# tepextepex/ENRGY

Measured on NVIDIA B200. Metric: cell-timesteps/s, higher is better.
Workload: dtype f32

## Files before the change

enrgy_b200/csrc/api.cu:

```cuda
#include <cuda_runtime.h>

#include <algorithm>
#include <cmath>
#include <cstdarg>
#include <cstdio>
#include <cstring>
#include <limits>
#include <string>
#include <thread>
#include <vector>

#include "../../include/enrgy_b200.h"
#include "common.cuh"
#include "kernels.cuh"
#include "prepass.cuh"

using namespace enrgy;

namespace {

thread_local std::string g_err;

int fail(int code, const char* fmt, ...) {
  char buf[1024];
// ... 138 lines not shown
  CU_TRY(cudaMemsetAsync(c->d_counters.p, 0, 2 * sizeof(unsigned long long), c->stream));
  CU_TRY(launch_mask_check(c->dem0, c->dem_pitch, d_other, c->pitch, c->band_row0, c->band_rows, c->cols,
                           c->d_counters.p, c->stream));
  c->launches++;
  unsigned long long h[2];
  CU_TRY(cudaMemcpyAsync(h, c->d_counters.p, sizeof(h), cudaMemcpyDeviceToHost, c->stream));
  CU_TRY(cudaStreamSynchronize(c->stream));
  if (h[0] != 0) {
    return fail(ENRGY_ERR_MASK,
                "%s is NaN at %llu cells where the DEM is valid; the reference would propagate NaN "
                "into only some of its area means there -- not supported",
                what, h[0]);
  }
  if (strict_other_valid && h[1] != 0) {
    return fail(ENRGY_ERR_MASK, "%s is valid at %llu cells where the DEM is NaN -- not supported", what,
                h[1]);
  }
  return ENRGY_OK;
}

template <typename R>
int upload_tables(enrgy_ctx* c) {
  const PrepassOutput& o = c->pre;
  const int T = c->n_steps;
  std::vector<StepRec<R>> st(T);
  for (int i = 0; i < T; ++i) {
    const StepRec<double>& s = o.steps[i];
    StepRec<R>& d = st[i];
    d.t_air = (R)s.t_air; d.lapse = (R)s.lapse; d.p_hpa = (R)s.p_hpa; d.e_aws = (R)s.e_aws;
    d.c_sens = (R)s.c_sens; d.c_lat = (R)s.c_lat; d.c_lwd = (R)s.c_lwd; d.c_lwu = (R)s.c_lwu;
    d.c_sw = (R)s.c_sw; d.c_melt = (R)s.c_melt; d.alb_w = (R)s.alb_w; d.snow_alb = (R)s.snow_alb;
    d.dsum = (R)s.dsum; d.dt = (R)s.dt; d.inv_dt = (R)s.inv_dt; d.c_lw0 = (R)s.c_lw0; d.c_lw1 = (R)s.c_lw1;
    d.dir_u = (R)s.dir_u; d.dir_e = (R)s.dir_e; d.dir_n = (R)s.dir_n;
    d.tan2_min = (R)s.tan2_min;
    if ((double)d.tan2_min > s.tan2_min) d.tan2_min = std::nextafter(d.tan2_min, (R)-1);
    const int32_t pair_code = (int32_t)s.alb_pair, sub_code = (int32_t)s.sub;
    d.alb_pair = (R)0; d.sub = (R)0;
    std::memcpy(&d.alb_pair, &pair_code, sizeof(int32_t));
    std::memcpy(&d.sub, &sub_code, sizeof(int32_t));
  }
  const size_t ns = o.subs.size();
  std::vector<SubRec<R>> sb(std::max<size_t>(ns, 1));
  for (size_t i = 0; i < ns; ++i) {
    sb[i].e = (R)o.subs[i].e; sb[i].n = (R)o.subs[i].n; sb[i].u = (R)o.subs[i].u; sb[i].b = (R)o.subs[i].b;
  }
  CU_TRY(c->d_steps.alloc(std::max<size_t>(T, 1) * sizeof(StepRec<R>)));
  CU_TRY(c->d_steps64.alloc(std::max<size_t>(T, 1)));
  CU_TRY(c->d_subs.alloc(sb.size() * sizeof(SubRec<R>)));
  CU_TRY(c->d_blocks.alloc(std::max<size_t>(o.blocks.size(), 1)));
  if (T) {
    CU_TRY(cudaMemcpyAsync(c->d_steps.p, st.data(), (size_t)T * sizeof(StepRec<R>), cudaMemcpyHostToDevice, c->stream));
    CU_TRY(cudaMemcpyAsync(c->d_steps64.p, o.steps.data(), (size_t)T * sizeof(StepRec<double>), cudaMemcpyHostToDevice, c->stream));
    CU_TRY(cudaMemcpyAsync(c->d_blocks.p, o.blocks.data(), o.blocks.size() * sizeof(TimeBlock), cudaMemcpyHostToDevice, c->stream));
  }
  if (ns) {
    CU_TRY(cudaMemcpyAsync(c->d_subs.p, sb.data(), ns * sizeof(SubRec<R>), cudaMemcpyHostToDevice, c->stream));
  }
  CU_TRY(cudaStreamSynchronize(c->stream));
  return ENRGY_OK;
}

template <typename R>
int upload_stations(enrgy_ctx* c) {
  const int T = c->n_steps;
  std::vector<StationRec<R>> recs((size_t)std::max(T, 1) * kMaxStations);
  for (int i = 0; i < T; ++i) {
    const StepRec<double>& s = c->pre.steps[i];
    StationRec<R>* r = &recs[(size_t)i * kMaxStations];
    r[0].t = (R)s.t_air; r[0].p = (R)s.p_hpa; r[0].e = (R)s.e_aws; r[0].cn = (R)0;
    const double n0 = c->forcing[(size_t)i * ENRGY_F_COUNT + ENRGY_F_CLOUD];
    for (int k = 1; k < kMaxStations; ++k) {
      if (k <= c->n_extra) {
// ... 1550 lines not shown
```

enrgy_b200/csrc/common.cuh:

```cuda
#pragma once
#include <cstdint>
#include <cmath>

#if defined(__CUDACC__)
#define ENRGY_HD __host__ __device__ __forceinline__
#else
#define ENRGY_HD inline
#endif

namespace enrgy {

constexpr double kRair = 287.058;
constexpr double kKarman = 0.4;
constexpr double kGrav = 9.81;
constexpr double kCpAir = 1010.0;
constexpr double kLv = 2.514 * 1e6;
constexpr double kSigma = 5.70 * 1e-8;
constexpr double kLf = 3.34 * 1e5;
constexpr double kCice = 2097.0;
constexpr double kKappaIce = 1.16 * 1e-6;
constexpr double kKappaSnow = 0.40 * 1e-6;
constexpr double kPressureLapse = -0.1145;
constexpr double kVapourScale = 6300.0;
constexpr double kMsmInitLapse = -0.006;

constexpr int kThreads = 256;
constexpr int kWarps = kThreads / 32;
constexpr int kTileW = 128;
constexpr int kStatsK = 8;
constexpr int kStatsM = 2;
constexpr int kStatsP = kStatsK + kStatsM;
#ifndef ENRGY_STEPS_PER_BLOCK
#define ENRGY_STEPS_PER_BLOCK 64
#endif
// ... 3 lines not shown
enum StatK { K_RS = 0, K_LWD, K_SENS, K_LAT, K_MELT, K_SNOW, K_SWE, K_NSNOW };
enum StatM { M_LWU = 0, M_G };

constexpr int kMaxLayers = 7;
template <typename R>
struct MsmParams {
  int layers;
  R d[kMaxLayers], inv_d[kMaxLayers];
  R c_ice, k_ice, k_snow, rho_ice, rho_snow;
  R inv_snow_density;
  R g0_ice;
  R crd_ice, inv_crd_ice;
};

template <typename R>
struct alignas(16) StepRec {
  R t_air;
  R lapse;
  R p_hpa;
  R e_aws;
  R c_sens;
  R c_lat;
  R c_lwd;
  R c_lwu;
  R c_sw;
  R c_melt;
  R alb_w;
  R snow_alb;
  R dsum;
  R dt;
  R alb_pair;
  R sub;
  R dir_u, dir_e, dir_n;
  R tan2_min;
  R inv_dt;
  R c_lw0;
  R c_lw1;
  R pad_;
};

constexpr int kMaxFusedMembers = 4;
template <typename R>
struct alignas(8) MemberRec {
  R c_sens, c_lat;
};

constexpr int kMaxStations = 4;
template <typename R>
struct alignas(16) StationRec {
  R t;
  R p;
  R e;
  R cn;
};

template <typename R>
struct alignas(16) SubRec {
  R e, n, u;
  R b;
};
struct alignas(16) ShadeRec {
  int32_t dc_fix;
  int32_t dr_fix;
  float dz;
  int32_t kmax;
};
ENRGY_HD void line_geometry(int dc_fix, int dr_fix, bool* row_type, int* sigma, int* dfix) {
  const int adr = dr_fix < 0 ? -dr_fix : dr_fix, adc = dc_fix < 0 ? -dc_fix : dc_fix;
  *row_type = adr >= adc;
  if (*row_type) { *sigma = dr_fix > 0 ? 1 : -1; *dfix = dc_fix; }
  else { *sigma = dc_fix > 0 ? 1 : -1; *dfix = dr_fix; }
}
// ... 9 lines not shown
```

enrgy_b200/csrc/kernels.cu:

```cuda
#include "kernels.cuh"

#include <cstdio>
#include <cstring>
#include <type_traits>

#include "../../include/enrgy_b200.h"

namespace enrgy {

__device__ __forceinline__ uint32_t smem_u32(const void* p) {
  return static_cast<uint32_t>(__cvta_generic_to_shared(p));
}
__device__ __forceinline__ void mbar_init(uint64_t* bar, unsigned count) {
  asm volatile("mbarrier.init.shared::cta.b64 [%0], %1;" ::"r"(smem_u32(bar)), "r"(count));
}
__device__ __forceinline__ void mbar_expect_tx(uint64_t* bar, unsigned bytes) {
  asm volatile("mbarrier.arrive.expect_tx.shared::cta.b64 _, [%0], %1;" ::"r"(smem_u32(bar)),
               "r"(bytes)
               : "memory");
}
__device__ __forceinline__ void mbar_wait(uint64_t* bar, unsigned parity) {
  asm volatile(
      "{\n\t"
      ".reg .pred p;\n\t"
// ... 102 lines not shown
  V2<float> d;
  asm("add.rn.f32x2 %0, %1, %2;" : "=l"(d.v) : "l"(a.v), "l"(b.v));
  return d;
}
__device__ __forceinline__ V2<float> sub2(V2<float> a, V2<float> b) {
  V2<float> d;
  asm("sub.rn.f32x2 %0, %1, %2;" : "=l"(d.v) : "l"(a.v), "l"(b.v));
  return d;
}
__device__ __forceinline__ V2<float> mul2(V2<float> a, V2<float> b) {
  V2<float> d;
  asm("mul.rn.f32x2 %0, %1, %2;" : "=l"(d.v) : "l"(a.v), "l"(b.v));
  return d;
}
__device__ __forceinline__ V2<double> fma2(V2<double> a, V2<double> b, V2<double> c) {
  return V2<double>{a.a * b.a + c.a, a.b * b.b + c.b};
}
__device__ __forceinline__ V2<double> add2(V2<double> a, V2<double> b) { return V2<double>{a.a + b.a, a.b + b.b}; }
__device__ __forceinline__ V2<double> sub2(V2<double> a, V2<double> b) { return V2<double>{a.a - b.a, a.b - b.b}; }
__device__ __forceinline__ V2<double> mul2(V2<double> a, V2<double> b) { return V2<double>{a.a * b.a, a.b * b.b}; }
__device__ __forceinline__ V2<float> lapse_product(V2<float> d, float g) {
  return V2<float>::make(__fmul_rn(d.lo(), g), __fmul_rn(d.hi(), g));
}
__device__ __forceinline__ V2<double> lapse_product(V2<double> d, double g) { return V2<double>{d.a * g, d.b * g}; }
__device__ __forceinline__ void keep_in_register(V2<float>& x) { asm volatile("" : "+l"(x.v)); }
__device__ __forceinline__ void keep_in_register(V2<double>&) {}

__device__ __forceinline__ float mul_rn(float a, float b) { return __fmul_rn(a, b); }
__device__ __forceinline__ float add_rn(float a, float b) { return __fadd_rn(a, b); }
__device__ __forceinline__ float div_rn(float a, float b) { return __fdiv_rn(a, b); }
__device__ __forceinline__ double mul_rn(double a, double b) { return __dmul_rn(a, b); }
__device__ __forceinline__ double add_rn(double a, double b) { return __dadd_rn(a, b); }
__device__ __forceinline__ double div_rn(double a, double b) { return __ddiv_rn(a, b); }
__device__ __forceinline__ float sq_sum(float x, float y) { return __fadd_rn(__fmul_rn(x, x), __fmul_rn(y, y)); }
__device__ __forceinline__ double sq_sum(double x, double y) { return __dadd_rn(__dmul_rn(x, x), __dmul_rn(y, y)); }

__device__ __forceinline__ float fmax_(float a, float b) { return fmaxf(a, b); }
__device__ __forceinline__ float fmin_(float a, float b) { return fminf(a, b); }
__device__ __forceinline__ double fmax_(double a, double b) { return fmax(a, b); }
__device__ __forceinline__ double fmin_(double a, double b) { return fmin(a, b); }

template <typename R>
__device__ __forceinline__ R warp_reduce8(const R (&v)[8], int lane) {
  const unsigned full = 0xffffffffu;
  R a[4], b[2], c;
  bool hi = (lane & 16) != 0;
#pragma unroll
  for (int i = 0; i < 4; ++i) {
    const R send = hi ? v[i] : v[i + 4];
    const R keep = hi ? v[i + 4] : v[i];
    a[i] = keep + __shfl_xor_sync(full, send, 16);
  }
  hi = (lane & 8) != 0;
#pragma unroll
  for (int i = 0; i < 2; ++i) {
    const R send = hi ? a[i] : a[i + 2];
    const R keep = hi ? a[i + 2] : a[i];
    b[i] = keep + __shfl_xor_sync(full, send, 8);
  }
  hi = (lane & 4) != 0;
  {
    const R send = hi ? b[0] : b[1];
    const R keep = hi ? b[1] : b[0];
    c = keep + __shfl_xor_sync(full, send, 4);
  }
  c += __shfl_xor_sync(full, c, 2);
  c += __shfl_xor_sync(full, c, 1);
  return c;
// ... 229 lines not shown
template <typename R>
cudaError_t launch_nan_offglacier(const float* dem, int dem_pitch, int pitch, int band_row0,
                                  int band_rows, int cols, R* swe, R* tsn, R* tic, cudaStream_t stream) {
  nan_offglacier_kernel<R><<<1184, 256, 0, stream>>>(dem, dem_pitch, pitch, band_row0, band_rows, cols, swe,
                                                     tsn, tic);
  return cudaGetLastError();
}
template cudaError_t launch_nan_offglacier<float>(const float*, int, int, int, int, int, float*, float*, float*, cudaStream_t);
template cudaError_t launch_nan_offglacier<double>(const float*, int, int, int, int, int, double*, double*, double*, cudaStream_t);

#ifndef ENRGY_WARPS32
#define ENRGY_WARPS32 4
#endif
#ifndef ENRGY_WARPS64
#define ENRGY_WARPS64 4
#endif
template <typename R, int INSOL>
constexpr int kWarpsFor = sizeof(R) == 4 ? ENRGY_WARPS32 : ENRGY_WARPS64;
__host__ __device__ constexpr int warps_x(int w) { return w >= 4 ? 4 : w; }

#ifndef ENRGY_MASK_RING
#define ENRGY_MASK_RING 0
#endif
constexpr int kRingSlots = 16, kRingAhead = 8;
__device__ __forceinline__ void cp_async16(void* smem_dst, const void* gsrc) {
  asm volatile("cp.async.cg.shared.global [%0], [%1], 16;" ::"r"(smem_u32(smem_dst)), "l"(gsrc) : "memory");
}
__device__ __forceinline__ void cp_async_commit() { asm volatile("cp.async.commit_group;" ::: "memory"); }
template <int N>
__device__ __forceinline__ void cp_async_wait() { asm volatile("cp.async.wait_group %0;" ::"n"(N) : "memory"); }

template <typename R>
struct SmemPlan {
  int steps, subs, members, stations, slots, slots_m, ring, full, total;
};
#ifndef ENRGY_ONE_BARRIER
#define ENRGY_ONE_BARRIER 1
#endif
template <typename R, bool MSM, int NM, int INSOL>
constexpr bool kOneBarrier = ENRGY_ONE_BARRIER && sizeof(R) == 4 && !MSM && NM == 1 && INSOL == kInsolMasked;

template <typename R>
__host__ __device__ inline SmemPlan<R> smem_plan(int warps, int cap_steps, int cap_subs, bool with_subs, bool msm,
                                                 int nm = 1, int ns = 1, bool with_masks = false) {
  SmemPlan<R> p;
  int o = 0;
  p.steps = o;   o += 2 * cap_steps * (int)sizeof(StepRec<R>);
  p.subs = o;    o += with_subs ? 2 * cap_subs * (int)sizeof(SubRec<R>) : 0;
  p.members = o; o += nm > 1 ? 2 * cap_steps * nm * (int)sizeof(MemberRec<R>) : 0;
  p.stations = o; o += ns > 1 ? 2 * cap_steps * ns * (int)sizeof(StationRec<R>) : 0;
  const bool two_sets = ENRGY_ONE_BARRIER && sizeof(R) == 4 && !msm && nm == 1 && with_masks;
  p.slots = o;   o += (two_sets ? 2 : 1) * warps * cap_steps * nm * kStatsK * (int)sizeof(R);
  p.slots_m = o; o += msm ? warps * cap_steps * kStatsM * (int)sizeof(R) : 0;
  o = (o + 15) / 16 * 16;
  p.ring = o;    o += (ENRGY_MASK_RING && with_masks) ? warps * kRingSlots * 32 : 0;
  p.full = o;    o += 16;
  p.total = (o + 127) / 128 * 128;
  return p;
}

#ifndef ENRGY_K32
#define ENRGY_K32 8
#endif
#ifndef ENRGY_K64
#define ENRGY_K64 4
#endif
#ifndef ENRGY_MINB32
#define ENRGY_MINB32 4
#endif
#ifndef ENRGY_MINB64
#define ENRGY_MINB64 3
#endif

#ifndef ENRGY_SUB_UNROLL
#define ENRGY_SUB_UNROLL 4
#endif
constexpr int kSubUnroll = ENRGY_SUB_UNROLL;
#ifndef ENRGY_MASK_AHEAD
#define ENRGY_MASK_AHEAD 4
#endif
constexpr int kMaskAhead = ENRGY_MASK_AHEAD;
#ifndef ENRGY_MINB_MEMBERS
#define ENRGY_MINB_MEMBERS 3
#endif
template <typename R, int K, int INSOL, bool MSM, bool DUMP, int NM = 1, int KT = K, bool STATS = true, int NS = 1>
__global__ void __launch_bounds__(32 * kWarpsFor<R, INSOL>, NM > 2 ? ENRGY_MINB_MEMBERS : sizeof(R) == 4 ? ENRGY_MINB32 : ENRGY_MINB64)
energy_balance_kernel(const KernelArgs<R> a) {
  static_assert(NM == 1 || (!MSM && !DUMP), "fused members: no sub-surface model, no dump");
  static_assert(KT % K == 0, "a patch is walked in whole parts");
  static_assert(STATS || NM > 1, "only fused members run without statistics");
  static_assert(NS == 1 || (NM == 1 && !MSM), "station blend: no fused members, no sub-surface model");
  constexpr int W = kWarpsFor<R, INSOL>;
  constexpr int WX = warps_x(W), WY = W / WX;
  constexpr int NT = 32 * W;
  extern __shared__ __align__(128) unsigned char smem_raw[];
  const int cap_steps = a.cap_steps, cap_subs = a.cap_subs;
  const SmemPlan<R> plan = smem_plan<R>(W, cap_steps, cap_subs, INSOL != kInsolStreamed, MSM, NM, NS, INSOL == kInsolMasked);
  StationRec<R>* const sm_stations = reinterpret_cast<StationRec<R>*>(smem_raw + plan.stations);
  StepRec<R>* const sm_steps = reinterpret_cast<StepRec<R>*>(smem_raw + plan.steps);
  SubRec<R>* const sm_subs = reinterpret_cast<SubRec<R>*>(smem_raw + plan.subs);
  MemberRec<R>* const sm_members = reinterpret_cast<MemberRec<R>*>(smem_raw + plan.members);
  R* const sm_slots0 = reinterpret_cast<R*>(smem_raw + plan.slots);
  constexpr bool ONE_BAR = kOneBarrier<R, MSM, NM, INSOL>;
  unsigned slot_set = 0;
  R* const sm_slots_m = reinterpret_cast<R*>(smem_raw + plan.slots_m);
  uint64_t* const sm_full = reinterpret_cast<uint64_t*>(smem_raw + plan.full);

  constexpr int TILE_H = WY * KT, TILE_W = 32 * WX;
  const int tid = threadIdx.x, lane = tid & 31, warp = tid >> 5;
  const R qnan = (R)__int_as_float(0x7fc00000);

  if (tid == 0) {
    mbar_init(&sm_full[0], 1);
    mbar_init(&sm_full[1], 1);
    fence_mbar_init();
  }
  __syncthreads();
  unsigned phase[2] = {0u, 0u};

  auto issue_block = [&](int b, int buf) {
    const TimeBlock tb = a.blocks[b];
    const unsigned n_steps = (unsigned)(tb.t_end - tb.t_begin);
    const unsigned n_subs = (unsigned)(tb.sub_end - tb.sub_begin);
    unsigned bytes = n_steps * (unsigned)sizeof(StepRec<R>);
    if (INSOL != kInsolStreamed) bytes += n_subs * (unsigned)sizeof(SubRec<R>);
    if (NM > 1) bytes += n_steps * NM * (unsigned)sizeof(MemberRec<R>);
    if (NS > 1) bytes += n_steps * NS * (unsigned)sizeof(StationRec<R>);
    fence_proxy_async();
    mbar_expect_tx(&sm_full[buf], bytes);
    tma_bulk_g2s(sm_steps + buf * cap_steps, a.steps + tb.t_begin, n_steps * (unsigned)sizeof(StepRec<R>),
// ... 83 lines not shown
        } else {
          x_[h] = y_[h] = (R)0; n_[h] = (R)1;
        }
#pragma unroll
        for (int m = 0; m < NM; ++m) {
          s_[m][h] = v ? a.swe[m * m_stride + o] : (R)0;
          t_[m][h] = v ? a.total_ice[m * m_stride + o] : (R)0;
        }
        if (MSM) {
#pragma unroll
          for (int l = 0; l < NB; ++l) {
            tl[i][l] = (v && l <= a.msm.layers) ? a.layer_t[(size_t)l * a.layer_stride + o] : (R)0;
          }
          t0_acc[i] = (double)tl[i][0];
        }
      }
      delta2[q] = V::make(d_[0], d_[1]);
      keep_in_register(delta2[q]);
#pragma unroll
      for (int k = 0; k < NS; ++k) {
        pw2[k][q] = V::make(p_[k][0], p_[k][1]);
        if (NS > 1) wst2[k][q] = V::make(w_[k][0], w_[k][1]);
      }
      nx2[q] = V::make(x_[0], x_[1]);
      ny2[q] = V::make(y_[0], y_[1]);
      nz2[q] = V::make(n_[0], n_[1]);
#pragma unroll
      for (int m = 0; m < NM; ++m) {
        swe2[m][q] = V::make(s_[m][0], s_[m][1]);
        tic2[m][q] = V::make(t_[m][0], t_[m][1]);
        om2[m][q] = V::splat(a.albedo_const ? (R)1 - m_alb_ice(m) : (R)0.5);
      }
    }
    constexpr bool kAnalyticBeam = INSOL == kInsolComputed && sizeof(R) == 4;
    R patch_g2 = (R)0;
    if (kAnalyticBeam) {
#pragma unroll
      for (int q = 0; q < KP; ++q) {
        patch_g2 = fmax_(patch_g2, fmax_(sq_sum(nx2[q].lo(), ny2[q].lo()), sq_sum(nx2[q].hi(), ny2[q].hi())));
      }
      if (KT > K) {
        const int prow0 = row0 - part * K;
        for (int i = 0; i < KT; ++i) {
          const int rowb = prow0 + i;
          if (rowb < a.band_rows && colx < a.cols && (i < part * K || i >= part * K + K)) {
            const size_t o = (size_t)rowb * a.pitch + colx;
            const R gx = a.nx[o], gy = a.ny[o];
            if (gx == gx) patch_g2 = fmax_(patch_g2, sq_sum(gx, gy));
          }
        }
      }
#pragma unroll
      for (int d = 16; d > 0; d >>= 1) patch_g2 = fmax_(patch_g2, __shfl_xor_sync(0xffffffffu, patch_g2, d));
      patch_g2 *= (R)1.00001;
    }
    keep_in_register(valid_bits);
    const bool patch_full = __all_sync(0xffffffffu, valid_bits == ((1u << K) - 1u));
    const unsigned lane_bit = 1u << lane;
    constexpr bool RING = ENRGY_MASK_RING && INSOL == kInsolMasked && K == 8;
    uint4* const ring = reinterpret_cast<uint4*>(smem_raw + plan.ring) + warp * kRingSlots * 2;
    int ring_next = -0x40000000;
    const unsigned* const mask_patch =
        INSOL == kInsolMasked
            ? a.masks + ((size_t)(row0 >> 3) * a.mask_words + (size_t)((colx - lane) >> 5)) * 8 + (row0 & 7) -
                  (size_t)a.mask_sub0 * a.mask_sub_stride
            : nullptr;

    int buf = 0;
    if (tid == 0) issue_block(a.block_begin, 0);

    for (int b = a.block_begin; b < a.block_end; ++b, buf ^= 1) {
      if (tid == 0 && b + 1 < a.block_end) issue_block(b + 1, buf ^ 1);
      R* const sm_slots = sm_slots0 + (ONE_BAR ? (size_t)(slot_set & 1u) * W * cap_steps * NM * kStatsK : 0);
      slot_set ^= 1u;
      mbar_wait(&sm_full[buf], phase[buf]);
      phase[buf] ^= 1u;
      const TimeBlock tb = a.blocks[b];
      const int ts = max(tb.t_begin, a.t0), te = min(tb.t_end, a.t1);

      float pot_next[K];
      if (INSOL == kInsolStreamed) {
#pragma unroll
        for (int i = 0; i < K; ++i) {
          const size_t o = (size_t)(ts - a.pot_t0) * a.pot_stride + (size_t)(row0 + i) * a.pitch + colx;
          pot_next[i] = (valid_bits >> i) & 1u ? __ldg(a.pot + o) : 0.f;
        }
      }

      auto run_steps = [&](auto full_tag) {
      constexpr bool FULL = decltype(full_tag)::value;
      const StepRec<R>* const steps_b = sm_steps + buf * cap_steps - tb.t_begin;
      int sub_next = step_code(steps_b[ts].sub), pair_next = step_code(steps_b[ts].alb_pair);
      R w_next = steps_b[ts].alb_w;
      for (int t = ts; t < te; ++t) {
        const StepRec<R> s = steps_b[t];
        const int sub_code = sub_next, pair = pair_next;
        const R alb_w = w_next;
        if (t + 1 < te) {
          sub_next = step_code(steps_b[t + 1].sub);
          pair_next = step_code(steps_b[t + 1].alb_pair);
          w_next = steps_b[t + 1].alb_w;
        }
        if (!a.albedo_const) {
          if (pair != cur_pair || alb_w != cur_w) {
            cur_pair = pair;
            cur_w = alb_w;
            const float* m0 = a.albedo + (size_t)(pair >> 8) * a.map_stride;
            const float* m1 = a.albedo + (size_t)(pair & 255) * a.map_stride;
#pragma unroll
            for (int q = 0; q < KP; ++q) {
              R om[NM][2];
#pragma unroll
              for (int h = 0; h < 2; ++h) {
                const int i = 2 * q + h;
                const size_t o = (size_t)(row0 + i) * a.pitch + colx;
                const bool v = (valid_bits >> i) & 1u;
                const R y0 = v ? (R)__ldg(m0 + o) : (R)0.5, y1 = v ? (R)__ldg(m1 + o) : (R)0.5;
#pragma unroll
                for (int m = 0; m < NM; ++m) {
                  const R x0 = v ? fmin_(fmax_(y0 + m_offset(m), (R)0.001f), (R)1) : (R)0.5;
                  const R x1 = v ? fmin_(fmax_(y1 + m_offset(m), (R)0.001f), (R)1) : (R)0.5;
                  om[m][h] = ((R)1 - x0) + alb_w * (x0 - x1);
                }
              }
#pragma unroll
              for (int m = 0; m < NM; ++m) om2[m][q] = V::make(om[m][0], om[m][1]);
            }
          }
        }
        float pot_cur[K];
        if (INSOL == kInsolStreamed) {
#pragma unroll
          for (int i = 0; i < K; ++i) pot_cur[i] = pot_next[i];
// ... 5 lines not shown
            }
          }
        }

        V pot2[KP];
        auto balance = [&]() {
        const V zero2 = V::splat((R)0);
        V acc_sens = zero2, acc_lat = zero2;
        V acc_lwd = zero2;
        V acc_rs[NM], acc_mf[NM], acc_snow[NM], acc_swe[NM], acc_lwu = zero2, acc_g = zero2;
        int n_snow[NM];
#pragma unroll
        for (int m = 0; m < NM; ++m) { acc_rs[m] = acc_mf[m] = acc_snow[m] = acc_swe[m] = zero2; n_snow[m] = 0; }
        const V keep_map = V::splat(s.snow_alb >= (R)0 ? (R)0 : (R)1);
        const R ice_floor = (R)1 - a.max_ice_albedo;
        const V t_aws = V::splat(s.t_air), lapse2 = V::splat(s.lapse), p_aws = V::splat(s.p_hpa), e_aws = V::splat(s.e_aws);
        const V c_lwd = V::splat(s.c_lwd), c_sw = V::splat(s.c_sw), c_melt = V::splat(s.c_melt);
        V c_sens[NM], c_lat[NM], snow_const[NM];
#pragma unroll
        for (int m = 0; m < NM; ++m) {
          if (NM > 1) {
            const MemberRec<R> mr = sm_members[(buf * cap_steps + (t - tb.t_begin)) * NM + m];
            c_sens[m] = V::splat(mr.c_sens);
            c_lat[m] = V::splat(mr.c_lat);
            const R sa = a.albedo_const ? a.member_albedo_snow[m] : s.snow_alb;
            snow_const[m] = V::splat(s.snow_alb >= (R)0 ? (R)1 - sa : (R)0);
          } else {
            c_sens[m] = V::splat(s.c_sens);
            c_lat[m] = V::splat(s.c_lat);
            snow_const[m] = V::splat(s.snow_alb >= (R)0 ? (R)1 - s.snow_alb : (R)0);
          }
        }
        const V k273 = V::splat((R)273.15), k_plapse = V::splat((R)kPressureLapse), k_rair = V::splat((R)kRair),
                k_fp0 = V::splat((R)1.0016), k_fp1 = V::splat((R)(3.15 * 1e-6)), k_fp2 = V::splat((R)-0.074);
#pragma unroll
        for (int q = 0; q < KP; ++q) {
          V t_st = t_aws, p_st = p_aws, e_st = zero2, cloud_fac = zero2;
          if (NS > 1) {
            const StationRec<R>* const sr = sm_stations + (buf * cap_steps + (t - tb.t_begin)) * NS;
            V cn = zero2;
#pragma unroll
            for (int k = 0; k < NS; ++k) {
              const StationRec<R> r = sr[k];
              if (k == 0) {
                t_st = sizeof(R) == 4 ? lapse_product(wst2[0][q], r.t) : mul2(wst2[0][q], V::splat(r.t));
                p_st = mul2(wst2[0][q], V::splat(r.p));
                e_st = mul2(pw2[0][q], V::splat(r.e));
              } else {
                t_st = sizeof(R) == 4 ? add2(t_st, lapse_product(wst2[k][q], r.t)) : fma2(wst2[k][q], V::splat(r.t), t_st);
                p_st = fma2(wst2[k][q], V::splat(r.p), p_st);
                e_st = fma2(pw2[k][q], V::splat(r.e), e_st);
                cn = k == 1 ? mul2(wst2[1][q], V::splat(r.cn)) : fma2(wst2[k][q], V::splat(r.cn), cn);
              }
            }
            if (a.cloud_on) {
              const V x = mul2(cn, V::splat(a.cloud_neg_k));
              cloud_fac = V::make(Num<R>::exp_(x.lo()), Num<R>::exp_(x.hi()));
            }
          }
          const V t_air = sizeof(R) == 4 ? add2(t_st, lapse_product(delta2[q], s.lapse)) : fma2(delta2[q], lapse2, t_st);
          const V tz = add2(t_air, k273);
          V d_t = sub2(tz, k273);
          if (MSM) {
            R d[2];
#pragma unroll
            for (int h = 0; h < 2; ++h) {
              const int i = 2 * q + h;
              const R tzh = h ? tz.hi() : tz.lo();
              d[h] = tzh - (tl[i][0] + (R)273.15);
              if (sizeof(R) == 4) {
                d[h] = ((tzh - (R)273.15) + (R)-6.103515625e-06) - tl[i][0];
              }
            }
            d_t = V::make(d[0], d[1]);
          }
          const V p_hpa = fma2(delta2[q], k_plapse, p_st);
          const V e = NS > 1 ? e_st : mul2(pw2[0][q], e_aws);
          V r_rt, r_p;
          {
            const V rt = mul2(tz, k_rair);
            if (sizeof(R) == 8) {
              const V den = mul2(rt, p_hpa);
              const V inv = V::make(Num<R>::rcp(den.lo()), Num<R>::rcp(den.hi()));
              r_rt = mul2(inv, p_hpa);
              r_p = mul2(inv, rt);
            } else {
              r_rt = V::make(Num<R>::rcp(rt.lo()), Num<R>::rcp(rt.hi()));
              r_p = V::make(Num<R>::rcp(p_hpa.lo()), Num<R>::rcp(p_hpa.hi()));
            }
          }
          const V x_sens = mul2(p_hpa, mul2(r_rt, d_t));
          const V f_p = fma2(r_p, k_fp2, fma2(p_hpa, k_fp1, k_fp0));
          V es_neg = V::splat((R)-611.2);
          if (MSM) {
            R x[2];
#pragma unroll
            for (int h = 0; h < 2; ++h) {
              const R t0 = tl[2 * q + h][0];
              x[h] = (R)-611.2 * Num<R>::exp_(((R)17.62 * t0) * Num<R>::rcp((R)243.12 + t0));
            }
            es_neg = V::make(x[0], x[1]);
          }
          const V x_lat = mul2(r_rt, fma2(es_neg, f_p, e));
          const V tzsq = mul2(tz, tz);
          const V tz4 = mul2(tzsq, tzsq);
          V lwu = V::splat(s.c_lwu);
          if (MSM) {
            R x[2];
#pragma unroll
            for (int h = 0; h < 2; ++h) {
              const R t0 = tl[2 * q + h][0];
              if (sizeof(R) == 4) {
                const R y = t0 * (R)(1.0 / 273.15);
                const R poly = (R)1 + y * ((R)4 + y * ((R)6 + y * ((R)4 + y)));
                x[h] = (s.c_lwu * (R)(273.15 * 273.15 * 273.15 * 273.15)) * poly;
              } else {
                const R ts_k = t0 + (R)273.15;
                const R ts2 = ts_k * ts_k;
                x[h] = s.c_lwu * (ts2 * ts2);
              }
            }
            lwu = V::make(x[0], x[1]);
          }
          V rl;
          if (sizeof(R) == 4 && !MSM) {
            const V y = mul2(d_t, V::splat((R)(1.0 / (double)273.15f)));
            const V poly = mul2(y, fma2(y, fma2(y, add2(y, V::splat((R)4)), V::splat((R)6)), V::splat((R)4)));
            rl = fma2(V::splat(s.c_lw1), poly, V::splat(s.c_lw0));
          } else {
            const V lwu_neg = V::make(-lwu.lo(), -lwu.hi());
            rl = fma2(c_lwd, tz4, lwu_neg);
          }
          const bool v_lo = (valid_bits >> (2 * q)) & 1u, v_hi = (valid_bits >> (2 * q + 1)) & 1u;
          if (STATS) {
            V m_sens = x_sens, m_lat = x_lat;
            if (!FULL) {
// ... 245 lines not shown
                  for (int p_ = 0; p_ < kRingAhead; ++p_) fetch(ms + p_);
                  ring_next = ms + kRingAhead;
                }
                fetch(ring_next);
                ++ring_next;
                cp_async_wait<kRingAhead>();
                __syncwarp();
                const uint4 m0 = ring[(ms & (kRingSlots - 1)) * 2], m1 = ring[(ms & (kRingSlots - 1)) * 2 + 1];
                mw[0] = m0.x; mw[1] = m0.y; mw[2 % K] = m0.z; mw[3 % K] = m0.w;
                mw[4 % K] = m1.x; mw[5 % K] = m1.y; mw[6 % K] = m1.z; mw[7 % K] = m1.w;
              } else if (K == 8) {
                const uint4 m0 = __ldg(reinterpret_cast<const uint4*>(mp)), m1 = __ldg(reinterpret_cast<const uint4*>(mp) + 1);
                mw[0] = m0.x; mw[1] = m0.y; mw[2 % K] = m0.z; mw[3 % K] = m0.w;
                mw[4 % K] = m1.x; mw[5 % K] = m1.y; mw[6 % K] = m1.z; mw[7 % K] = m1.w;
              } else if (K == 4) {
                const uint4 m0 = __ldg(reinterpret_cast<const uint4*>(mp));
                mw[0] = m0.x; mw[1] = m0.y; mw[2 % K] = m0.z; mw[3 % K] = m0.w;
              } else {
                const uint2 m0 = __ldg(reinterpret_cast<const uint2*>(mp));
                mw[0] = m0.x; mw[1] = m0.y;
              }
            }
#pragma unroll
            for (int q = 0; q < KP; ++q) {
              R c_lo = fmax_(c2[q].lo(), (R)0), c_hi = fmax_(c2[q].hi(), (R)0);
              if (INSOL == kInsolMasked) {
                c_lo = (mw[2 * q] & lane_bit) ? c_lo : (R)0;
                c_hi = (mw[2 * q + 1] & lane_bit) ? c_hi : (R)0;
              }
              direct2[q] = fma2(b2, V::make(c_lo, c_hi), direct2[q]);
            }
          };
          constexpr bool kOneBalance = MSM;
          if (kAnalyticBeam && patch_g2 < s.tan2_min) {
            const V du = V::splat(s.dir_u), de = V::splat(s.dir_e), dn = V::splat(s.dir_n);
#pragma unroll
            for (int q = 0; q < KP; ++q) direct2[q] = fma2(ny2[q], dn, fma2(nx2[q], de, du));
            if (!kOneBalance) finish_step();
          } else if (nj == 4) {
            sub_step(j0); sub_step(j0 + 1); sub_step(j0 + 2); sub_step(j0 + 3);
            if (!kOneBalance) finish_step();
          } else {
#pragma unroll(kSubUnroll)
            for (int j = j0; j < j0 + nj; ++j) sub_step(j);
            if (!kOneBalance) finish_step();
          }
          if (kOneBalance) finish_step();
        }
      }
      };
      if (patch_full) run_steps(std::true_type{}); else run_steps(std::false_type{});

      __syncthreads();
      if (!DUMP && STATS && my_partials != nullptr) {
        constexpr int NQ = MSM ? kStatsP : kStatsK;
        const int n = (te - ts) * NM * NQ;
        for (int idx = tid; idx < n; idx += NT) {
          const int step = idx / NQ, q = idx - step * NQ;
          const int sl = (ts - tb.t_begin) * NM + step;
          double sum = 0.0;
#pragma unroll
          for (int w = 0; w < W; ++w) {
            sum += q < kStatsK ? (double)sm_slots[(w * cap_steps * NM + sl) * kStatsK + q]
                               : (double)sm_slots_m[(w * cap_steps + sl) * kStatsM + (q - kStatsK)];
          }
          my_partials[((size_t)(ts - a.t0) * NM + step) * kRow + q] += (R)sum;
        }
// ... 27 lines not shown
        }
      }
    }
  }
}

template <typename R, bool MSM>
struct CellsPerThread {
  static constexpr int kBase = sizeof(R) == 4 ? ENRGY_K32 : ENRGY_K64;
  static constexpr int value = MSM ? ((kBase / 2 + 1) & ~1) : kBase;
};

template <typename R>
void energy_balance_tile(bool msm, int insol, int* tile_h, int* tile_w) {
  const int k = msm ? CellsPerThread<R, true>::value : CellsPerThread<R, false>::value;
  (void)insol;
  const int w = kWarpsFor<R, kInsolComputed>;
  *tile_w = 32 * warps_x(w);
  *tile_h = (w / warps_x(w)) * k;
}
template void energy_balance_tile<float>(bool, int, int*, int*);
template void energy_balance_tile<double>(bool, int, int*, int*);

template <typename R, bool MSM, int NM, int NS = 1>
struct PassShape {
  static constexpr int KT = CellsPerThread<R, MSM>::value;
  static constexpr int K = (NM > 1 || NS > 1) ? KT / 2 : KT;
};

template <typename R, int INSOL, bool MSM, bool DUMP, int NM = 1, bool STATS = true, int NS = 1>
static cudaError_t configure(int sm_count, int cap_steps, int cap_subs, LaunchInfo* info) {
  constexpr int K = PassShape<R, MSM, NM, NS>::K, KT = PassShape<R, MSM, NM, NS>::KT;
  auto kern = energy_balance_kernel<R, K, INSOL, MSM, DUMP, NM, KT, STATS, NS>;
  const int smem = smem_plan<R>(kWarpsFor<R, INSOL>, cap_steps, cap_subs, INSOL != kInsolStreamed, MSM, NM, NS, INSOL == kInsolMasked).total;
  cudaError_t e = cudaFuncSetAttribute(kern, cudaFuncAttributeMaxDynamicSharedMemorySize, smem);
  if (e != cudaSuccess) return e;
  int per_sm = 0;
  e = cudaOccupancyMaxActiveBlocksPerMultiprocessor(&per_sm, kern, 32 * kWarpsFor<R, INSOL>, smem);
  if (e != cudaSuccess) return e;
  cudaFuncAttributes fa;
  e = cudaFuncGetAttributes(&fa, kern);
  if (e != cudaSuccess) return e;
  if (per_sm < 1) per_sm = 1;
  info->regs = fa.numRegs;
  info->smem_bytes = smem;
  info->ctas_per_sm = per_sm;
  info->grid = per_sm * sm_count;
  info->cells_per_thread = K;
  return cudaSuccess;
}

template <typename R, int INSOL, bool MSM, bool DUMP, int NM = 1, bool STATS = true, int NS = 1>
static cudaError_t launch_one(const KernelArgs<R>& a, int sm_count, int forced_grid, LaunchInfo* info,
                              cudaStream_t stream) {
  constexpr int K = PassShape<R, MSM, NM, NS>::K, KT = PassShape<R, MSM, NM, NS>::KT;
  LaunchInfo li;
  cudaError_t e = configure<R, INSOL, MSM, DUMP, NM, STATS, NS>(sm_count, a.cap_steps, a.cap_subs, &li);
  if (e != cudaSuccess) return e;
  int grid = forced_grid > 0 ? forced_grid : li.grid;
  li.grid = grid;
  if (info) *info = li;
  if (a.n_tiles == 0 || a.t1 <= a.t0) return cudaSuccess;
  energy_balance_kernel<R, K, INSOL, MSM, DUMP, NM, KT, STATS, NS><<<grid, 32 * kWarpsFor<R, INSOL>, li.smem_bytes, stream>>>(a);
  return cudaGetLastError();
}

template <typename R, typename F>
// ... 326 lines not shown
```

enrgy_b200/csrc/prepass.cu:

```cuda
#include "prepass.cuh"

#include <algorithm>
#include <cmath>
#include <cstdio>
#include <limits>

namespace enrgy {

namespace {

constexpr double kDeg = 0.017453292519943295;
constexpr double kPi = 3.141592653589793;

constexpr double kA = 0.7, kB = 0.75, kC = 5.0, kD = 0.35;

double minus_psi_m(double z, double l) {
  const double zeta = z / l;
  if (zeta >= 0) {
    return kA * zeta + kB * (zeta - kC / kD) * std::exp(-kD * zeta) + kB * kC / kD;
  }
  const double x = std::pow(1 - 16 * zeta, 0.25);
  return -(2 * std::log((1 + x) / 2) + std::log((1 + x * x) / 2) - 2 * std::atan(x) + kPi / 2);
}

// ... 228 lines not shown
    } else {
      s.c_lwu = p.emissivity * kSigma * std::pow(ts_k, 4.0);
    }
    {
      const double k0 = (double)273.15f, k04 = (k0 * k0) * (k0 * k0);
      const double c_lwd_k = mirror32 ? (double)(float)s.c_lwd : s.c_lwd;
      s.c_lw1 = c_lwd_k * k04;
      s.c_lw0 = s.c_lw1 - (mirror32 ? (double)(float)s.c_lwu : s.c_lwu);
    }
    s.c_melt = dt / kLf / 1000;
    s.dt = dt;
    s.inv_dt = 1.0 / dt;

    const int i0 = (int)f[ENRGY_F_ALB_I0], i1 = (int)f[ENRGY_F_ALB_I1];
    const double span = f[ENRGY_F_ALB_SPAN];
    s.alb_pair = (double)(i0 * 256 + i1);
    s.alb_w = span > 0 ? f[ENRGY_F_ALB_DAYS] / span : 0.0;
    const double snow_days = f[ENRGY_F_SNOW_DAYS];
    s.snow_alb = snow_days > 0 ? 0.40 + 0.44 * std::exp(-0.12 * snow_days) : -1.0;
    if (p.albedo_const) {
      s.snow_alb = p.albedo_snow;
      s.alb_w = 0.0;
      s.alb_pair = 0.0;
    }

    double pot_aws_kwh = 0.0;
    out.sub_first[i] = (int)out.subs.size();
    if (computed) {
      const double dt_h = dt / 3600.0;
      const double hs = p.hour_step;
      int n_sub = (int)std::ceil(dt_h / hs - 1e-9);
      if (n_sub < 1) n_sub = 1;
      double direct = 0.0, dsum = 0.0;
      double dir_u = 0.0, dir_e = 0.0, dir_n = 0.0, tan2_min = std::numeric_limits<double>::infinity();
      for (int j = 0; j < n_sub; ++j) {
        const double w = std::min(hs, dt_h - j * hs);
        const double t_mid = f[ENRGY_F_TIME] + (j * hs + 0.5 * w) * 3600.0;
        SubHost sb;
        sun_vector(t_mid, p.lat_deg, p.lon_deg, &sb.e, &sb.n, &sb.u);
        if (!(sb.u > 0.0)) continue;
        const double tb = std::pow(p.transmittance, 1.0 / sb.u);
        sb.b = p.solar_const * tb * w / 1000.0;
        sb.d = p.solar_const * (0.271 - 0.294 * tb) * sb.u * w / 1000.0 * 0.5;
        const double m = std::max(std::fabs(sb.e), std::fabs(sb.n));
        if (m > 0.0) {
          sb.shade.dc_fix = (int32_t)std::floor(sb.e / m * 65536.0 + 0.5);
          sb.shade.dr_fix = (int32_t)std::floor(-sb.n / m * 65536.0 + 0.5);
          sb.shade.dz = (float)(p.cell_size * sb.u / m);
        } else {
          sb.shade.dc_fix = 0;
          sb.shade.dr_fix = 0;
          sb.shade.dz = std::numeric_limits<float>::infinity();
        }
        sb.shade.kmax = std::max(in.rows, in.cols);
        out.subs.push_back(sb);
        dir_u += sb.b * sb.u; dir_e += sb.b * sb.e; dir_n += sb.b * sb.n;
        {
          const double h2 = sb.e * sb.e + sb.n * sb.n;
          if (h2 > 0.0) tan2_min = std::min(tan2_min, sb.u * sb.u / h2);
        }
        const double cosi = nx * sb.e + ny * sb.n + nz * sb.u;
        double term = sb.b * std::max(cosi, 0.0);
        if (p.shadow && !host_lit(in.dem, in.rows, in.cols, p.aws_row, p.aws_col, sb.shade)) {
          term = 0.0;
        }
        direct = direct + term;
        dsum = dsum + sb.d;
      }
      s.dsum = dsum;
      s.dir_u = dir_u; s.dir_e = dir_e; s.dir_n = dir_n;
      s.tan2_min = (int)out.subs.size() == out.sub_first[i] ? -1.0 : std::min(tan2_min, 1e30);
      pot_aws_kwh = direct + dsum * (1.0 + nz);
    } else {
      s.dsum = 0.0;
      s.dir_u = s.dir_e = s.dir_n = 0.0; s.tan2_min = -1.0;
      pot_aws_kwh = in.pot_aws ? in.pot_aws[i] : 0.0;
    }
    out.sub_count[i] = (int)out.subs.size() - out.sub_first[i];
    if (out.sub_count[i] > 255) {
      err = "more than 255 insolation sub-steps in one time step";
      return ENRGY_ERR_RANGE;
    }

    double pot_w, factor;
    const double swd = f[ENRGY_F_SWD];
    if (mirror32 && !computed) {
      const float pw32 = (((float)pot_aws_kwh * 3.6f) * 1000000.0f) / (float)dt;
      pot_w = (double)pw32;
      factor = pw32 == 0.0f ? 1.0 : (double)((float)swd / pw32);
    } else {
      pot_w = pot_aws_kwh * 3.6 * 1000000 / dt;
      factor = pot_w == 0 ? 1.0 : swd / pot_w;
    }
    s.c_sw = 3.6 * 1000000 / dt * factor;

    const double t_air_c = t_air + delta_cell * f[ENRGY_F_LAPSE];
    const double tz_c = t_air_c + 273.15;
    const double tsk = ts_aws_c + 273.15;
    const double p_c = p_hpa + delta_cell * kPressureLapse;
    const double r_rt = 1.0 / (kRair * tz_c);
    const double sens = (s.c_sens * p_c) * (r_rt * (tz_c - tsk));
    const double f_p = 1.0016 + 3.15 * 1e-6 * p_c - 0.074 / p_c;
    const double es = 611.2 * std::exp((17.62 * ts_aws_c) / (243.12 + ts_aws_c)) * f_p;
    const double lat = (s.c_lat * r_rt) * (e_aws * pw_cell - es);
    pt[ENRGY_P_SENS_AWS] = sens;
    pt[ENRGY_P_LAT_AWS] = lat;
    if (msm) {
      for (int lyr = 0; lyr <= nl; ++lyr) out.point_layers[(size_t)i * (kMaxLayers + 1) + lyr] = tl[lyr];
// ... 82 lines not shown
```

Measured before the change: 579.0 billion.

## Use per-azimuth-sector slope bounds to take analytic beam path more often

Replaces the single patch-wide max-gradient test for skipping the shadow ray march with a per-warp table of directional slope maxima over 64 azimuth sectors at 6 arc widths. The prepass encodes each step's sun-azimuth arc as a sector code and stores the min sun tangent (not its square). The tighter bound lets more timesteps take the cheap analytic direct-beam path, at the cost of a per-warp table build and extra shared memory. It also refolds the latent-heat vapour pressure terms into fused multiply-adds for the non-MSM path.

After: 610.2 billion, median of 6. 5.4% higher.

```diff
diff --git a/enrgy_b200/csrc/api.cu b/enrgy_b200/csrc/api.cu
--- a/enrgy_b200/csrc/api.cu
+++ b/enrgy_b200/csrc/api.cu
@@ -194,12 +194,13 @@
     d.c_sw = (R)s.c_sw; d.c_melt = (R)s.c_melt; d.alb_w = (R)s.alb_w; d.snow_alb = (R)s.snow_alb;
     d.dsum = (R)s.dsum; d.dt = (R)s.dt; d.inv_dt = (R)s.inv_dt; d.c_lw0 = (R)s.c_lw0; d.c_lw1 = (R)s.c_lw1;
     d.dir_u = (R)s.dir_u; d.dir_e = (R)s.dir_e; d.dir_n = (R)s.dir_n;
-    d.tan2_min = (R)s.tan2_min;
-    if ((double)d.tan2_min > s.tan2_min) d.tan2_min = std::nextafter(d.tan2_min, (R)-1);
-    const int32_t pair_code = (int32_t)s.alb_pair, sub_code = (int32_t)s.sub;
-    d.alb_pair = (R)0; d.sub = (R)0;
+    d.tan_min = (R)s.tan_min;
+    if ((double)d.tan_min > s.tan_min) d.tan_min = std::nextafter(d.tan_min, (R)-1);
+    const int32_t pair_code = (int32_t)s.alb_pair, sub_code = (int32_t)s.sub, sector_code = (int32_t)s.sector;
+    d.alb_pair = (R)0; d.sub = (R)0; d.sector = (R)0;
     std::memcpy(&d.alb_pair, &pair_code, sizeof(int32_t));
     std::memcpy(&d.sub, &sub_code, sizeof(int32_t));
+    std::memcpy(&d.sector, &sector_code, sizeof(int32_t));
   }
   const size_t ns = o.subs.size();
   std::vector<SubRec<R>> sb(std::max<size_t>(ns, 1));
diff --git a/enrgy_b200/csrc/common.cuh b/enrgy_b200/csrc/common.cuh
--- a/enrgy_b200/csrc/common.cuh
+++ b/enrgy_b200/csrc/common.cuh
@@ -1,5 +1,6 @@
 #pragma once
 #include <cstdint>
+#include <algorithm>
 #include <cmath>
 
 #if defined(__CUDACC__)
@@ -69,12 +70,27 @@
   R alb_pair;
   R sub;
   R dir_u, dir_e, dir_n;
-  R tan2_min;
+  R tan_min;
   R inv_dt;
   R c_lw0;
   R c_lw1;
-  R pad_;
+  R sector;
 };
+
+constexpr int kSectors = 64;
+constexpr int kSectorLevels = 6;
+inline int sector_arc_code(const int* sec, int n) {
+  if (n <= 0) return -1;
+  int best_len = kSectors + 1, best_first = 0;
+  for (int i = 0; i < n; ++i) {
+    int len = 0;
+    for (int j = 0; j < n; ++j) len = std::max(len, ((sec[j] - sec[i]) % kSectors + kSectors) % kSectors + 1);
+    if (len < best_len) { best_len = len; best_first = sec[i]; }
+  }
+  int level = 0;
+  while ((1 << level) < best_len) ++level;
+  return level < kSectorLevels ? level * kSectors + best_first : -1;
+}
 
 constexpr int kMaxFusedMembers = 4;
 template <typename R>
diff --git a/enrgy_b200/csrc/kernels.cu b/enrgy_b200/csrc/kernels.cu
--- a/enrgy_b200/csrc/kernels.cu
+++ b/enrgy_b200/csrc/kernels.cu
@@ -158,8 +158,6 @@
 __device__ __forceinline__ double mul_rn(double a, double b) { return __dmul_rn(a, b); }
 __device__ __forceinline__ double add_rn(double a, double b) { return __dadd_rn(a, b); }
 __device__ __forceinline__ double div_rn(double a, double b) { return __ddiv_rn(a, b); }
-__device__ __forceinline__ float sq_sum(float x, float y) { return __fadd_rn(__fmul_rn(x, x), __fmul_rn(y, y)); }
-__device__ __forceinline__ double sq_sum(double x, double y) { return __dadd_rn(__dmul_rn(x, x), __dmul_rn(y, y)); }
 
 __device__ __forceinline__ float fmax_(float a, float b) { return fmaxf(a, b); }
 __device__ __forceinline__ float fmin_(float a, float b) { return fminf(a, b); }
@@ -455,17 +453,20 @@
 
 template <typename R>
 struct SmemPlan {
-  int steps, subs, members, stations, slots, slots_m, ring, full, total;
+  int steps, subs, members, stations, slots, slots_m, ring, sectors, full, total;
 };
 #ifndef ENRGY_ONE_BARRIER
 #define ENRGY_ONE_BARRIER 1
 #endif
+template <typename R, int INSOL>
+constexpr bool kAnalyticBeamFor = INSOL == kInsolComputed && sizeof(R) == 4;
 template <typename R, bool MSM, int NM, int INSOL>
 constexpr bool kOneBarrier = ENRGY_ONE_BARRIER && sizeof(R) == 4 && !MSM && NM == 1 && INSOL == kInsolMasked;
 
 template <typename R>
 __host__ __device__ inline SmemPlan<R> smem_plan(int warps, int cap_steps, int cap_subs, bool with_subs, bool msm,
-                                                 int nm = 1, int ns = 1, bool with_masks = false) {
+                                                 int nm = 1, int ns = 1, bool with_masks = false,
+                                                 bool with_sectors = false) {
   SmemPlan<R> p;
   int o = 0;
   p.steps = o;   o += 2 * cap_steps * (int)sizeof(StepRec<R>);
@@ -477,6 +478,7 @@
   p.slots_m = o; o += msm ? warps * cap_steps * kStatsM * (int)sizeof(R) : 0;
   o = (o + 15) / 16 * 16;
   p.ring = o;    o += (ENRGY_MASK_RING && with_masks) ? warps * kRingSlots * 32 : 0;
+  p.sectors = o; o += with_sectors ? warps * kSectorLevels * kSectors * (int)sizeof(float) : 0;
   p.full = o;    o += 16;
   p.total = (o + 127) / 128 * 128;
   return p;
@@ -518,7 +520,8 @@
   constexpr int NT = 32 * W;
   extern __shared__ __align__(128) unsigned char smem_raw[];
   const int cap_steps = a.cap_steps, cap_subs = a.cap_subs;
-  const SmemPlan<R> plan = smem_plan<R>(W, cap_steps, cap_subs, INSOL != kInsolStreamed, MSM, NM, NS, INSOL == kInsolMasked);
+  const SmemPlan<R> plan = smem_plan<R>(W, cap_steps, cap_subs, INSOL != kInsolStreamed, MSM, NM, NS, INSOL == kInsolMasked,
+                                        kAnalyticBeamFor<R, INSOL>);
   StationRec<R>* const sm_stations = reinterpret_cast<StationRec<R>*>(smem_raw + plan.stations);
   StepRec<R>* const sm_steps = reinterpret_cast<StepRec<R>*>(smem_raw + plan.steps);
   SubRec<R>* const sm_subs = reinterpret_cast<SubRec<R>*>(smem_raw + plan.subs);
@@ -668,27 +671,66 @@
         om2[m][q] = V::splat(a.albedo_const ? (R)1 - m_alb_ice(m) : (R)0.5);
       }
     }
-    constexpr bool kAnalyticBeam = INSOL == kInsolComputed && sizeof(R) == 4;
-    R patch_g2 = (R)0;
-    if (kAnalyticBeam) {
-#pragma unroll
-      for (int q = 0; q < KP; ++q) {
-        patch_g2 = fmax_(patch_g2, fmax_(sq_sum(nx2[q].lo(), ny2[q].lo()), sq_sum(nx2[q].hi(), ny2[q].hi())));
+    constexpr bool kAnalyticBeam = kAnalyticBeamFor<R, INSOL>;
+    float* const sec_tab = reinterpret_cast<float*>(smem_raw + plan.sectors) + warp * kSectorLevels * kSectors;
+    if constexpr (kAnalyticBeam) {
+      constexpr int KO = KT - K;
+      float ox[KO > 0 ? KO : 1], oy[KO > 0 ? KO : 1];
+#pragma unroll
+      for (int j = 0; j < KO; ++j) {
+        const int i = j < part * K ? j : j + K;
+        const int rowb = row0 - part * K + i;
+        ox[j] = oy[j] = 0.f;
+        if (rowb < a.band_rows && colx < a.cols) {
+          const size_t o = (size_t)rowb * a.pitch + colx;
+          const float gx = a.nx[o], gy = a.ny[o];
+          if (gx == gx) { ox[j] = gx; oy[j] = gy; }
+        }
       }
-      if (KT > K) {
-        const int prow0 = row0 - part * K;
-        for (int i = 0; i < KT; ++i) {
-          const int rowb = prow0 + i;
-          if (rowb < a.band_rows && colx < a.cols && (i < part * K || i >= part * K + K)) {
-            const size_t o = (size_t)rowb * a.pitch + colx;
-            const R gx = a.nx[o], gy = a.ny[o];
-            if (gx == gx) patch_g2 = fmax_(patch_g2, sq_sum(gx, gy));
-          }
-        }
+      float hb_lo = 0.f, hb_hi = 0.f;
+      for (int i = 0; i < kSectors / 2; ++i) {
+        float sn, cs;
+        sincospif((float)i * (2.0f / kSectors), &sn, &cs);
+        float dmin = 0.f, dmax = 0.f;
+#pragma unroll
+        for (int q = 0; q < KP; ++q) {
+          const float d0 = fmaf(nx2[q].lo(), cs, ny2[q].lo() * sn), d1 = fmaf(nx2[q].hi(), cs, ny2[q].hi() * sn);
+          dmin = fminf(dmin, fminf(d0, d1));
+          dmax = fmaxf(dmax, fmaxf(d0, d1));
+        }
+#pragma unroll
+        for (int j = 0; j < KO; ++j) {
+          const float d = fmaf(ox[j], cs, oy[j] * sn);
+          dmin = fminf(dmin, d);
+          dmax = fmaxf(dmax, d);
+        }
+#pragma unroll
+        for (int d = 16; d > 0; d >>= 1) {
+          dmin = fminf(dmin, __shfl_xor_sync(0xffffffffu, dmin, d));
+          dmax = fmaxf(dmax, __shfl_xor_sync(0xffffffffu, dmax, d));
+        }
+        if (lane == i) { hb_lo = -dmin; hb_hi = dmax; }
       }
-#pragma unroll
-      for (int d = 16; d > 0; d >>= 1) patch_g2 = fmax_(patch_g2, __shfl_xor_sync(0xffffffffu, patch_g2, d));
-      patch_g2 *= (R)1.00001;
+      auto shifted = [&](float lo, float hi, int d, float* out_lo, float* out_hi) {
+        const float x = __shfl_sync(0xffffffffu, lo, (lane + d) & 31), y = __shfl_sync(0xffffffffu, hi, (lane + d) & 31);
+        const bool wrap = lane + d >= 32;
+        *out_lo = wrap ? y : x;
+        *out_hi = wrap ? x : y;
+      };
+      const float scale = (float)(1.0001 / cos(M_PI / kSectors));
+      float m_lo = hb_lo, m_hi = hb_hi;
+      __syncwarp();
+#pragma unroll
+      for (int lv = 0; lv < kSectorLevels; ++lv) {
+        float h_lo, h_hi, n_lo, n_hi;
+        shifted(hb_lo, hb_hi, 1 << lv, &h_lo, &h_hi);
+        sec_tab[lv * kSectors + lane] = fmaxf(m_lo, h_lo) * scale;
+        sec_tab[lv * kSectors + lane + 32] = fmaxf(m_hi, h_hi) * scale;
+        shifted(m_lo, m_hi, 1 << lv, &n_lo, &n_hi);
+        m_lo = fmaxf(m_lo, n_lo);
+        m_hi = fmaxf(m_hi, n_hi);
+      }
+      __syncwarp();
     }
     keep_in_register(valid_bits);
     const bool patch_full = __all_sync(0xffffffffu, valid_bits == ((1u << K) - 1u));
@@ -727,14 +769,16 @@
       constexpr bool FULL = decltype(full_tag)::value;
       const StepRec<R>* const steps_b = sm_steps + buf * cap_steps - tb.t_begin;
       int sub_next = step_code(steps_b[ts].sub), pair_next = step_code(steps_b[ts].alb_pair);
+      int sec_next = kAnalyticBeam ? step_code(steps_b[ts].sector) : 0;
       R w_next = steps_b[ts].alb_w;
       for (int t = ts; t < te; ++t) {
         const StepRec<R> s = steps_b[t];
-        const int sub_code = sub_next, pair = pair_next;
+        const int sub_code = sub_next, pair = pair_next, sec_code = sec_next;
         const R alb_w = w_next;
         if (t + 1 < te) {
           sub_next = step_code(steps_b[t + 1].sub);
           pair_next = step_code(steps_b[t + 1].alb_pair);
+          if (kAnalyticBeam) sec_next = step_code(steps_b[t + 1].sector);
           w_next = steps_b[t + 1].alb_w;
         }
         if (!a.albedo_const) {
@@ -806,10 +850,12 @@
           }
         }
         const V k273 = V::splat((R)273.15), k_plapse = V::splat((R)kPressureLapse), k_rair = V::splat((R)kRair),
-                k_fp0 = V::splat((R)1.0016), k_fp1 = V::splat((R)(3.15 * 1e-6)), k_fp2 = V::splat((R)-0.074);
+                k_fp0 = V::splat((R)1.0016), k_fp1 = V::splat((R)(3.15 * 1e-6)), k_fp2 = V::splat((R)-0.074),
+                k_es0 = V::splat((R)(-611.2 * 1.0016)), k_es1 = V::splat((R)(-611.2 * 3.15e-6)),
+                k_es2 = V::splat((R)(611.2 * 0.074));
 #pragma unroll
         for (int q = 0; q < KP; ++q) {
-          V t_st = t_aws, p_st = p_aws, e_st = zero2, cloud_fac = zero2;
+          V t_st = t_aws, p_st = p_aws, cloud_fac = zero2;
           if (NS > 1) {
             const StationRec<R>* const sr = sm_stations + (buf * cap_steps + (t - tb.t_begin)) * NS;
             V cn = zero2;
@@ -819,11 +865,9 @@
               if (k == 0) {
                 t_st = sizeof(R) == 4 ? lapse_product(wst2[0][q], r.t) : mul2(wst2[0][q], V::splat(r.t));
                 p_st = mul2(wst2[0][q], V::splat(r.p));
-                e_st = mul2(pw2[0][q], V::splat(r.e));
               } else {
                 t_st = sizeof(R) == 4 ? add2(t_st, lapse_product(wst2[k][q], r.t)) : fma2(wst2[k][q], V::splat(r.t), t_st);
                 p_st = fma2(wst2[k][q], V::splat(r.p), p_st);
-                e_st = fma2(pw2[k][q], V::splat(r.e), e_st);
                 cn = k == 1 ? mul2(wst2[1][q], V::splat(r.cn)) : fma2(wst2[k][q], V::splat(r.cn), cn);
               }
             }
@@ -849,7 +893,6 @@
             d_t = V::make(d[0], d[1]);
           }
           const V p_hpa = fma2(delta2[q], k_plapse, p_st);
-          const V e = NS > 1 ? e_st : mul2(pw2[0][q], e_aws);
           V r_rt, r_p;
           {
             const V rt = mul2(tz, k_rair);
@@ -864,18 +907,29 @@
             }
           }
           const V x_sens = mul2(p_hpa, mul2(r_rt, d_t));
-          const V f_p = fma2(r_p, k_fp2, fma2(p_hpa, k_fp1, k_fp0));
-          V es_neg = V::splat((R)-611.2);
+          V e_es;
           if (MSM) {
+            const V e = mul2(pw2[0][q], e_aws);
+            const V f_p = fma2(r_p, k_fp2, fma2(p_hpa, k_fp1, k_fp0));
             R x[2];
 #pragma unroll
             for (int h = 0; h < 2; ++h) {
               const R t0 = tl[2 * q + h][0];
               x[h] = (R)-611.2 * Num<R>::exp_(((R)17.62 * t0) * Num<R>::rcp((R)243.12 + t0));
             }
-            es_neg = V::make(x[0], x[1]);
-          }
-          const V x_lat = mul2(r_rt, fma2(es_neg, f_p, e));
+            e_es = fma2(V::make(x[0], x[1]), f_p, e);
+          } else {
+            V x = fma2(p_hpa, k_es1, k_es0);
+            if (NS > 1) {
+              const StationRec<R>* const sr = sm_stations + (buf * cap_steps + (t - tb.t_begin)) * NS;
+#pragma unroll
+              for (int k = 0; k < NS; ++k) x = fma2(pw2[k][q], V::splat(sr[k].e), x);
+            } else {
+              x = fma2(pw2[0][q], e_aws, x);
+            }
+            e_es = fma2(r_p, k_es2, x);
+          }
+          const V x_lat = mul2(r_rt, e_es);
           const V tzsq = mul2(tz, tz);
           const V tz4 = mul2(tzsq, tzsq);
           V lwu = V::splat(s.c_lwu);
@@ -1187,7 +1241,7 @@
             }
           };
           constexpr bool kOneBalance = MSM;
-          if (kAnalyticBeam && patch_g2 < s.tan2_min) {
+          if (kAnalyticBeam && sec_tab[sec_code] < s.tan_min) {
             const V du = V::splat(s.dir_u), de = V::splat(s.dir_e), dn = V::splat(s.dir_n);
 #pragma unroll
             for (int q = 0; q < KP; ++q) direct2[q] = fma2(ny2[q], dn, fma2(nx2[q], de, du));
@@ -1281,7 +1335,8 @@
 static cudaError_t configure(int sm_count, int cap_steps, int cap_subs, LaunchInfo* info) {
   constexpr int K = PassShape<R, MSM, NM, NS>::K, KT = PassShape<R, MSM, NM, NS>::KT;
   auto kern = energy_balance_kernel<R, K, INSOL, MSM, DUMP, NM, KT, STATS, NS>;
-  const int smem = smem_plan<R>(kWarpsFor<R, INSOL>, cap_steps, cap_subs, INSOL != kInsolStreamed, MSM, NM, NS, INSOL == kInsolMasked).total;
+  const int smem = smem_plan<R>(kWarpsFor<R, INSOL>, cap_steps, cap_subs, INSOL != kInsolStreamed, MSM, NM, NS, INSOL == kInsolMasked,
+                                kAnalyticBeamFor<R, INSOL>).total;
   cudaError_t e = cudaFuncSetAttribute(kern, cudaFuncAttributeMaxDynamicSharedMemorySize, smem);
   if (e != cudaSuccess) return e;
   int per_sm = 0;
diff --git a/enrgy_b200/csrc/prepass.cu b/enrgy_b200/csrc/prepass.cu
--- a/enrgy_b200/csrc/prepass.cu
+++ b/enrgy_b200/csrc/prepass.cu
@@ -284,7 +284,8 @@
       int n_sub = (int)std::ceil(dt_h / hs - 1e-9);
       if (n_sub < 1) n_sub = 1;
       double direct = 0.0, dsum = 0.0;
-      double dir_u = 0.0, dir_e = 0.0, dir_n = 0.0, tan2_min = std::numeric_limits<double>::infinity();
+      double dir_u = 0.0, dir_e = 0.0, dir_n = 0.0, tan_min = std::numeric_limits<double>::infinity();
+      std::vector<int> sectors;
       for (int j = 0; j < n_sub; ++j) {
         const double w = std::min(hs, dt_h - j * hs);
         const double t_mid = f[ENRGY_F_TIME] + (j * hs + 0.5 * w) * 3600.0;
@@ -309,7 +310,11 @@
         dir_u += sb.b * sb.u; dir_e += sb.b * sb.e; dir_n += sb.b * sb.n;
         {
           const double h2 = sb.e * sb.e + sb.n * sb.n;
-          if (h2 > 0.0) tan2_min = std::min(tan2_min, sb.u * sb.u / h2);
+          if (h2 > 0.0) {
+            tan_min = std::min(tan_min, sb.u / std::sqrt(h2));
+            const double turns = std::atan2(sb.n, sb.e) / (2.0 * M_PI);
+            sectors.push_back(((int)std::floor(turns * kSectors) % kSectors + kSectors) % kSectors);
+          }
         }
         const double cosi = nx * sb.e + ny * sb.n + nz * sb.u;
         double term = sb.b * std::max(cosi, 0.0);
@@ -321,11 +326,14 @@
       }
       s.dsum = dsum;
       s.dir_u = dir_u; s.dir_e = dir_e; s.dir_n = dir_n;
-      s.tan2_min = (int)out.subs.size() == out.sub_first[i] ? -1.0 : std::min(tan2_min, 1e30);
+      const int arc = sector_arc_code(sectors.data(), (int)sectors.size());
+      const bool sunlit = (int)out.subs.size() > out.sub_first[i];
+      s.sector = arc < 0 ? 0.0 : (double)arc;
+      s.tan_min = !sunlit || (arc < 0 && !sectors.empty()) ? -1.0 : std::min(tan_min, 1e30);
       pot_aws_kwh = direct + dsum * (1.0 + nz);
     } else {
       s.dsum = 0.0;
-      s.dir_u = s.dir_e = s.dir_n = 0.0; s.tan2_min = -1.0;
+      s.dir_u = s.dir_e = s.dir_n = 0.0; s.tan_min = -1.0; s.sector = 0.0;
       pot_aws_kwh = in.pot_aws ? in.pot_aws[i] : 0.0;
     }
     out.sub_count[i] = (int)out.subs.size() - out.sub_first[i];
```
